# renjie-liang/HUAL

Hardware: AMD Instinct MI355X
Metric: train clips/sec (higher is better)
Workload: dtype f32 (fp16x3 / bf16x3 split-operand MFMA, fp32 accumulate); 1 GPU; Charades-STA SeqPAN train step (fwd+bwd+clip+AdamWD, dropout 0.2), batch 64/GPU, T=128, vdim=1024, L=20, C=8, dim=128, 8 heads, 2 attention layers, random init; ONE batch resident in HBM, batch assembly (hual_assemble_batch) outside the timed region; global_batch=64, T=128, vdim=1024, L=20, parallelism=dp1, launch=hipGraph, video_dtype=f32

## Files before the change

### hual_amd/csrc/embed.h

```cpp
#pragma once
#include "common.h"
#include "embed_args.h"
#include "gemm.h"

namespace hual {

struct EmbedLayout { int CP; size_t cemb, ball, yall, dxall, dfall, total; };
EmbedLayout embed_layout(int nrows, int C, int char_dim);
int embed_cpad(int char_dim);
int embed_gather_tasks(const EmbedArgs& a, int nrows);
int launch_embed_fwd(const EmbedArgs& a, int nrows, const DropCfg& drop, hipStream_t s);
void embed_dw_job(const EmbedArgs& a, int nrows, DwJob* dwjob);
int launch_embed_bwd(const EmbedArgs& a, const EmbedGrads& g, int nrows, const DropCfg& drop, hipStream_t s, DwJob* dwjob, bool finish = true);
int embed_finish_blocks(const EmbedArgs& a, int nrows);
int embed_finish_lds(const EmbedArgs& a);
int launch_embed_unpack(const EmbedArgs& a, const EmbedGrads& g, hipStream_t s);
int embed_unpack_tasks(const EmbedArgs& a);
int embed_unpack_cpad(const EmbedArgs& a);

}
```

### hual_amd/csrc/embed.hip

```cpp
#include "embed.h"
#include "mproj.h"
#include "philox.h"
#include "prof.h"

using namespace hual;

#include "embed_gather.h"

namespace hual {
static inline int cpad(int char_dim) { return (char_dim + 15) / 16 * 16; }
EmbedLayout embed_layout(int nrows, int C, int char_dim) {
  EmbedLayout l;
  const int CP = cpad(char_dim);
  const size_t M = (size_t)nrows * C;
  l.CP = CP;
  size_t off = 0;
  l.cemb = off; off += (M + 4) * CP;
  l.ball = off; off += NALL;
  l.yall = off; off += M * NALL;
  l.dxall = off; off += M * 4 * CP;
  l.dfall = off; off += (size_t)4 * CP * NALL + NALL;
  l.total = off;
  return l;
}
}

__global__ __launch_bounds__(256) void char_pool_kernel(EmbedArgs a, int nrows) {
  const int gid = blockIdx.x * 256 + threadIdx.x;
  if (gid >= nrows * NCH) return;
  const int row = gid / NCH, ch = gid - row * NCH;
  int k, chk;
  chan_to_kernel(ch, k, chk);
  const float* y = a.yall + (size_t)row * a.C * NALL + ch;
  float best = 0.f;
  int arg = -1;
  for (int p = 0; p + k <= a.C; ++p) {
    const float v = y[(size_t)p * NALL];
    if (v > best) { best = v; arg = p; }
  }
  a.cat[(size_t)row * a.ldcat + a.word_dim + ch] = best;
  a.char_arg[(size_t)row * NCH + ch] = arg;
}

__global__ __launch_bounds__(256) void char_pool_bwd_kernel(EmbedArgs a, EmbedGrads gr, DropCfg drop, int nrows, int CP,
                                                            int ntask_pool) {
  const int gid = blockIdx.x * 256 + threadIdx.x;
  const int C = a.C, wd = a.word_dim;
  if (gid < ntask_pool) {
    const int row = gid / NALL, col = gid - row * NALL;
    int arg = -1;
    float g = 0.f;
    if (col < NCH) {
      arg = a.char_arg[(size_t)row * NCH + col];
      if (arg >= 0) g = gr.dcat[(size_t)row * gr.lddcat + wd + col];
    }
    float* y = a.yall + (size_t)row * C * NALL + col;
    for (int p = 0; p < C; ++p) y[(size_t)p * NALL] = p == arg ? g : 0.f;
    return;
  }
  int x = gid - ntask_pool;
  const int ngw = wd >> 2;
  if (x < nrows * ngw) {
    const int row = x / ngw, c4 = x - row * ngw;
    const int wid = a.word_ids[row];
    float* dst = nullptr;
    if (wid == 1) dst = gr.dunk;
    else if (wid >= 2 && wid - 2 < gr.dword_rows) dst = gr.dword_table + (size_t)(wid - 2) * wd;
    if (dst) {
      float4 g = ld4(gr.dcat + (size_t)row * gr.lddcat + 4 * c4);
      if (drop.enabled) g = apply_drop4(drop, HUAL_SITE_WORD, (uint32_t)row, (uint32_t)c4, g);
      atomicAdd(dst + 4 * c4, g.x); atomicAdd(dst + 4 * c4 + 1, g.y);
      atomicAdd(dst + 4 * c4 + 2, g.z); atomicAdd(dst + 4 * c4 + 3, g.w);
    }
    return;
  }
  x -= nrows * ngw;
  if (x < 4 * CP * NALL + NALL) a.dfall[x] = 0.f;
}

__global__ __launch_bounds__(256) void embed_finish_kernel(EmbedArgs a, EmbedGrads gr, DropCfg drop, int nrows, int CP) {
  extern __shared__ float dT[];
  embed_finish_block(a, gr, drop, nrows, CP, blockIdx.x, dT);
}

__global__ __launch_bounds__(256) void embed_unpack_kernel(EmbedArgs a, EmbedGrads gr, int CP) {
  embed_unpack_task(a, gr, CP, blockIdx.x * 256 + threadIdx.x);
}

namespace hual {

static int check_args(const EmbedArgs& a) {
  HUAL_REQUIRE(a.C >= 4, "char_ids need at least 4 chars per word (conv width 4, VALID) - modules.py:33");
  HUAL_REQUIRE((a.word_dim % 4) == 0 && a.char_dim >= 1, "embed: word_dim must be a multiple of 4");
  HUAL_REQUIRE(a.cemb && a.wall_img && a.ball && a.yall && a.dxall && a.dfall, "embed: null scratch");
  return 0;
}

int embed_cpad(int char_dim) { return cpad(char_dim); }
int embed_gather_tasks(const EmbedArgs& a, int nrows) {
  const int CP = cpad(a.char_dim);
  return nrows * (a.word_dim / 4 + a.C * (CP / 4)) + 4 * CP + NALL;
}

int launch_embed_fwd(const EmbedArgs& a, int nrows, const DropCfg& drop, hipStream_t s) {
  int rc = check_args(a);
  if (rc) return rc;
  const int CP = cpad(a.char_dim);
  MProjArgs g{};
  g.R = nrows * a.C; g.MT = mproj_rows(g.R); g.nsteps = 1;
  MProjStep& st = g.s[0];
  st.A = a.cemb; st.lda = CP; st.rep = cdiv(4 * CP, 128); st.ktot = 4 * CP; st.kw = 4 * CP < 128 ? 4 * CP : 128; st.wimg = a.wall_img; st.wrows = 4 * CP;
  st.first = 1; st.last = 1; st.drop_site = -1; st.add_div = 1;
  st.bias = a.ball; st.out = a.yall; st.ldo = NALL; st.ncol = NALL;
  const int C = a.C;
  const int mtp = (g.MT + C - 1) / C * C;
  if ((C & (C - 1)) == 0 && C <= 16 && mtp <= 64) {
    g.MT = mtp;
    st.out = nullptr;
    g.pool_cat = a.cat; g.pool_ldcat = a.ldcat; g.pool_col0 = a.word_dim; g.pool_arg = a.char_arg; g.pool_C = C;
    return launch_mproj(&g, 1, drop, s);
  }
  rc = launch_mproj(&g, 1, drop, s);
  if (rc) return rc;
  HUAL_LAUNCH(0.0, 0.0, char_pool_kernel, dim3(cdiv(nrows * NCH, 256)), dim3(256), 0, s, a, nrows);
  HUAL_CHECK_HIP(hipGetLastError());
  return 0;
}

int embed_finish_blocks(const EmbedArgs& a, int nrows) { return cdiv(nrows * a.C, EF_ROWS); }
int embed_finish_lds(const EmbedArgs& a) { return (a.num_chars - 1) * a.char_dim * (int)sizeof(float); }
int launch_embed_bwd(const EmbedArgs& a, const EmbedGrads& g, int nrows, const DropCfg& drop, hipStream_t s, DwJob* dwjob, bool finish) {
  int rc = check_args(a);
  if (rc) return rc;
  HUAL_REQUIRE(dwjob != nullptr, "embed_bwd: null weight-gradient job");
  const int cd = a.char_dim, CP = cpad(cd), M = nrows * a.C;
  const int ntask_pool = nrows * NALL;
  const int ntail = nrows * (a.word_dim / 4) + 4 * CP * NALL + NALL;
  HUAL_LAUNCH(0.0, 0.0, char_pool_bwd_kernel, dim3(cdiv(ntask_pool + ntail, 256)), dim3(256), 0, s, a, g, drop, nrows, CP,
              ntask_pool);
  HUAL_CHECK_HIP(hipGetLastError());
  embed_dw_job(a, nrows, dwjob);
  HUAL_REQUIRE(a.wall_img_t != nullptr && cdiv(4 * CP, 128) <= MP_MAX, "embed_bwd: image of the transposed filter bank");
  MProjArgs j{};
  j.R = M; j.MT = mproj_rows(M); j.nsteps = cdiv(4 * CP, 128);
  for (int p = 0; p < j.nsteps; ++p) {
    MProjStep& st = j.s[p];
    st.A = a.yall; st.lda = NALL; st.kw = NALL; st.reuse = p > 0 ? 1 : 0; st.rep = 1;
    st.wimg = reinterpret_cast<const float*>(reinterpret_cast<const char*>(a.wall_img_t) + (size_t)p * HUAL_PACK_BLOCK_BYTES); st.wrows = NALL;
    st.first = 1; st.last = 1; st.drop_site = -1; st.add_div = 1;
    st.out = a.dxall + (size_t)p * 128; st.ldo = 4 * CP; st.ncol = 4 * CP - 128 * p < 128 ? 4 * CP - 128 * p : 128;
  }
  rc = launch_mproj(&j, 1, drop, s);
  if (rc) return rc;
  const size_t lds = (size_t)(a.num_chars - 1) * cd * sizeof(float);
  HUAL_REQUIRE(lds <= 64 * 1024, "embed_bwd: char table too large for the LDS accumulator");
  if (!finish) return 0;
  HUAL_LAUNCH(0.0, 0.0, embed_finish_kernel, dim3(cdiv(M, EF_ROWS)), dim3(256), lds, s, a, g, drop, nrows, CP);
  HUAL_CHECK_HIP(hipGetLastError());
  return 0;
}

void embed_dw_job(const EmbedArgs& a, int nrows, DwJob* dwjob) {
  const int CP = cpad(a.char_dim);
  dw_job_init(*dwjob);
  dwjob->npieces = 1;
  dwjob->A[0] = a.cemb; dwjob->lda[0] = CP; dwjob->kw[0] = 4 * CP; dwjob->dW[0] = a.dfall; dwjob->ldw = NALL;
  dwjob->dY = a.yall; dwjob->ldy = NALL; dwjob->M = nrows * a.C; dwjob->N = NALL;
  dwjob->db = a.dfall + (size_t)4 * CP * NALL;
}

int embed_unpack_tasks(const EmbedArgs& a) { return a.char_dim * 300 + NCH; }
int embed_unpack_cpad(const EmbedArgs& a) { return cpad(a.char_dim); }
int launch_embed_unpack(const EmbedArgs& a, const EmbedGrads& g, hipStream_t s) {
  const int cd = a.char_dim;
  const int n = cd * 300 + NCH;
  HUAL_LAUNCH(0.0, 0.0, embed_unpack_kernel, dim3(cdiv(n, 256)), dim3(256), 0, s, a, g, cpad(cd));
  HUAL_CHECK_HIP(hipGetLastError());
  return 0;
}

}
```

### hual_amd/csrc/embed_args.h

```cpp
#pragma once
#include "common.h"

namespace hual {

struct EmbedArgs {
  const int32_t* word_ids;
  const int32_t* char_ids;
  const float* word_table;
  const float* unk;
  const float* char_table;
  const float* filt[4];
  const float* fbias[4];
  float* cat; int ldcat;
  int32_t* char_arg;
  int word_dim, char_dim, C, num_chars;
  float* cemb; float* ball; float* yall; float* dxall; float* dfall;
  const float* wall_img; const float* wall_img_t;
};
struct EmbedGrads {
  const float* dcat; int lddcat;
  float* dunk; float* dchar_table; float* dfilt[4]; float* dfbias[4];
  float* dword_table; int dword_rows;
};

}
```

### hual_amd/csrc/prof.cpp

```cpp
#include <stdlib.h>
#include "prof.h"
#include <map>
#include <string>
#include <vector>
#include <string.h>
#include "../../include/hual_seqpan.h"

namespace hual {

namespace {
struct Rec { std::string name; hipEvent_t a, b; double flops, bytes; };
struct Agg { std::string name; int64_t launches = 0; double usec = 0.0, flops = 0.0, bytes = 0.0; };
struct State {
  bool on = false;
  std::vector<Rec> recs;
  std::vector<Agg> aggs;
};
thread_local State g_prof;

std::string clean(const char* s) {
  std::string n(s);
  while (!n.empty() && (n.front() == '(' || n.front() == ' ')) n.erase(n.begin());
  while (!n.empty() && (n.back() == ')' || n.back() == ' ')) n.pop_back();
  return n;
}
}

bool prof_on() { return g_prof.on; }
bool lds_poison_on() {
  static const bool on = getenv("HUAL_DEBUG_LDS_POISON") != nullptr && atoi(getenv("HUAL_DEBUG_LDS_POISON")) != 0;
  return on;
}

void prof_events(const char* name, double flops, double bytes, hipEvent_t* start, hipEvent_t* stop) {
  *start = *stop = nullptr;
  hipEvent_t a, b;
  if (hipEventCreate(&a) != hipSuccess) return;
  if (hipEventCreate(&b) != hipSuccess) { hipEventDestroy(a); return; }
  g_prof.recs.push_back(Rec{clean(name), a, b, flops, bytes});
  *start = a;
  *stop = b;
}

}

extern "C" {

int hual_prof_begin(void) {
  hual::g_prof.on = true;
  hual::g_prof.recs.clear();
  hual::g_prof.aggs.clear();
  return 0;
}

int hual_prof_end(void) {
  using namespace hual;
  g_prof.on = false;
  std::map<std::string, size_t> idx;
  g_prof.aggs.clear();
  for (auto& r : g_prof.recs) {
    hipEventSynchronize(r.b);
    float ms = 0.f;
    const bool ok = hipEventElapsedTime(&ms, r.a, r.b) == hipSuccess;
    auto it = idx.find(r.name);
    if (it == idx.end()) {
      it = idx.emplace(r.name, g_prof.aggs.size()).first;
      g_prof.aggs.push_back(Agg{r.name});
    }
    Agg& a = g_prof.aggs[it->second];
    if (ok) { a.launches += 1; a.usec += (double)ms * 1e3; a.flops += r.flops; a.bytes += r.bytes; }
    hipEventDestroy(r.a);
    hipEventDestroy(r.b);
  }
  g_prof.recs.clear();
  return (int)g_prof.aggs.size();
}

int hual_prof_get(int i, char* name, int name_cap, int64_t* launches, double* usec, double* flops, double* bytes) {
  using namespace hual;
  if (i < 0 || i >= (int)g_prof.aggs.size() || !name || name_cap < 1) return HUAL_ERR_INVALID;
  const Agg& a = g_prof.aggs[i];
  strncpy(name, a.name.c_str(), (size_t)name_cap - 1);
  name[name_cap - 1] = 0;
  if (launches) *launches = a.launches;
  if (usec) *usec = a.usec;
  if (flops) *flops = a.flops;
  if (bytes) *bytes = a.bytes;
  return 0;
}

int hual_prof_kernel_pipe(const char* kernel, int* pipe, int* passes) {
  if (!kernel || !pipe || !passes) return HUAL_ERR_INVALID;
  struct Row { const char* prefix; int pipe, passes; };
  static const Row rows[] = {
      {"conv_block_", HUAL_PIPE_MATRIX16, 3}, {"ln_proj", HUAL_PIPE_MATRIX16, 3}, {"da_post", HUAL_PIPE_MATRIX16, 3},
      {"da_mid_bwd", HUAL_PIPE_MATRIX16, 3},  {"ln2_mid_bwd", HUAL_PIPE_MATRIX16, 3}, {"mproj_", HUAL_PIPE_MATRIX16, 3},
      {"feature_", HUAL_PIPE_MATRIX16, 3},    {"dw_f16_", HUAL_PIPE_MATRIX16, 3},
      {"attn_", HUAL_PIPE_MATRIX16, 3},      {"cq_fwd_staged", HUAL_PIPE_MATRIX16, 3}, {"cq_bwd_staged", HUAL_PIPE_MATRIX16, 3},
      {"cq_fwd_wide", HUAL_PIPE_MATRIX16, 3}, {"cq_bwd_wide", HUAL_PIPE_MATRIX16, 3},
      {"cq_", HUAL_PIPE_MATRIX32, 1},
  };
  for (const Row& r : rows)
    if (strncmp(kernel, r.prefix, strlen(r.prefix)) == 0) { *pipe = r.pipe; *passes = r.passes; return 0; }
  *pipe = HUAL_PIPE_NONE; *passes = 0;
  return 0;
}

}
```

### hual_amd/csrc/seqpan.hip

```cpp
#include "attn.h"
#include "prof.h"
#include "cq.h"
#include "convblock.h"
#include "dablock.h"
#include "embed.h"
#include "gemm.h"
#include "heads.h"
#include "mproj.h"
#include "optim.h"
#include "params.h"
#include "rowops.h"
#include <stdlib.h>
#include <string.h>
#include <algorithm>
#include <unordered_map>
#include <vector>

namespace hual {
const char* last_error_cstr();
}
using namespace hual;

namespace {

// ... 377 lines not shown
  AlignPool& ap = f.align;
  ap.F2 = cqf; ap.F1 = cqf; ap.inner = (lab && !c.dry) ? lab->inner_labels : nullptr;
  ap.tpre = r("align.tpre", B, D); ap.vpre = r("align.vpre", B, D);
  ap.that = r("align.tv", B, 2 * D); ap.vhat = ap.that + D; ap.ld = 2 * D;
  f.fuse = r.actv("fuse"); f.outputs = r.actv("outputs");
  f.probs = r("match.probs", c.rs.Nv, 4); f.match_part = r("match.part", (size_t)match_fwd_blocks(c.rs.Nv), 2);
  f.d_that = r("d.align.that", B, D); f.d_vhat = r("d.align.vhat", B, D);
  f.align_scratch = r("align.scratch", (size_t)2 * B, B); f.align_rows = r("align.rowloss", B, 1);
  return f;
}
MatchArgs match_args(const Ctx& c, const CoreBufs& k, const FuseBufs& f, const hual_labels* lab, const hual_run_opts* opt) {
  MatchArgs ma{};
  ma.fuse = f.fuse; ma.Wm = c.p(c.pm.match.k); ma.bm = c.p(c.pm.match.b); ma.E = c.p(c.pm.label_emb);
  ma.labels = (lab && !c.dry) ? lab->match_labels : nullptr;
  ma.outputs = f.outputs; ma.loss_acc = k.loss_acc;
  if (!c.cfg->no_gumbel) { ma.rng = opt->rng_state; ma.inv_tau = 1.0f / c.cfg->tau; }
  return ma;
}

struct FeBufs {
  float *x0, *a, *mean, *rstd, *qkv; uint8_t* kb4;
  CbBufs cb;
  float* att; AttnJob job; float *res, *l2, *mean2, *rstd2, *out; uint8_t *kb6, *kb7, *kb8;
};
FeBufs fe_bufs(const Res& r, int ps) {
  const Ctx& c = r.c;
  const int D = HUAL_D, Nv = c.rs.Nv;
  const std::string t = "fe" + std::to_string(ps);
  FeBufs b{};
  b.x0 = r.actv(t + ".x0"); b.a = r.actv(t + ".a");
  b.mean = r(t + ".ln1.mean", Nv, 1); b.rstd = r(t + ".ln1.rstd", Nv, 1);
  b.qkv = r(t + ".qkv", Nv, 3 * D); b.kb4 = r.bits(t + ".kb4", Nv);
  b.cb = cb_bufs(r, t, b.x0, Nv);
  b.att = r.actv(t + ".att");
  AttnJob& a = b.job;
  attn_job_init(a);
  a.Q = b.qkv; a.ldq = 3 * D; a.K = b.qkv + D; a.V = b.qkv + 2 * D; a.ldkv = 3 * D; a.O = b.att; a.ldo = D;
  a.B = c.B; a.Tq = c.T; a.Tk = c.T; a.qrow0 = 0; a.krow0 = 0; a.qmask = c.rs.rowmask; a.kmask = c.rs.rowmask;
  a.drop_site = HUAL_SITE_FE + 16 * ps + 5;
  set_dmask(r, a, t + ".dm");
  b.res = r.actv(t + ".res"); b.l2 = r.actv(t + ".l2");
  b.mean2 = r(t + ".ln2.mean", Nv, 1); b.rstd2 = r(t + ".ln2.rstd", Nv, 1);
  b.out = r.actv(t + ".out");
  b.kb6 = r.bits(t + ".kb6", Nv); b.kb7 = r.bits(t + ".kb7", Nv); b.kb8 = r.bits(t + ".kb8", Nv);
  return b;
}

struct HeadBufs { float *fn[2], *mean, *rstd, *h[2], *d_logit[2], *dz[2], *part[2], *loc_part; };
HeadBufs head_bufs(const Res& r) {
  const Ctx& c = r.c;
  const int D = HUAL_D, Nv = c.rs.Nv, B = c.B;
  HeadBufs b{};
  b.fn[0] = r.actv("head.sfn"); b.fn[1] = r.actv("head.efn");
  b.mean = r("head.mean", (size_t)2 * Nv, 1); b.rstd = r("head.rstd", (size_t)2 * Nv, 1);
  b.h[0] = r.actv("head.hs"); b.h[1] = r.actv("head.he");
  b.d_logit[0] = r("d.s_logit", B, c.T); b.d_logit[1] = r("d.e_logit", B, c.T);
  b.dz[0] = r.actv("d.head.zs"); b.dz[1] = r.actv("d.head.ze");
  b.part[0] = r("head.part.s", (size_t)B * 2, D); b.part[1] = r("head.part.e", (size_t)B * 2, D);
  b.loc_part = r("loc.part", B, 1);
  return b;
}

void fill_da_ln_proj(Ctx& c, LnProjArgs& lp, int li) {
  const int D = HUAL_D;
  const DualAttnP& d = c.pm.da[li];
  const DaLnBufs n = da_ln_bufs(Res{c, true}, li);
  lp = LnProjArgs{};
  lp.g1 = c.p(d.ln1.g); lp.b1 = c.p(d.ln1.b); lp.y1 = n.ln1; lp.drop_site1 = -1; lp.pre_site = -1;
  lp.g2 = c.p(d.lnt.g); lp.b2 = c.p(d.lnt.b); lp.y2 = n.lnt; lp.mean = n.mean; lp.rstd = n.rstd;
  lp.nproj = 5; lp.R = c.rs.R; lp.Nv = c.rs.Nv; lp.MT = ln_proj_rows(c.rs.R, c.rs.Nv); lp.drop_row0 = 0;
  const DenseP* pr[5] = {&d.query, &d.f_key, &d.f_value, &d.t_key, &d.t_value};
  float* outs[5] = {n.qkv, n.qkv + D, n.qkv + 2 * D, n.ktvt, n.ktvt + D};
  for (int k = 0; k < 5; ++k) {
    lp.wimg[k] = c.timg(pr[k]->k); lp.bias[k] = c.p(pr[k]->b); lp.out[k] = outs[k]; lp.ldo[k] = k < 3 ? 3 * D : 2 * D; lp.src[k] = k < 3 ? 0 : 1;
    lp.out_site[k] = -1;
  }
}

bool cb_no_tail() {
  static const bool no_tail = getenv("HUAL_CB_NO_TAIL") != nullptr && atoi(getenv("HUAL_CB_NO_TAIL")) != 0;
  return no_tail;
}

float* conv_block_fwd(Ctx& c, const CbBufs& b, const ConvBlockP& cp, const RowSpace& rs, int site0,
                      const float* pos_src = nullptr, const float* pos = nullptr, LnProjArgs* tail = nullptr, bool* tail_done = nullptr) {
  CbFwdArgs a{};
  a.x0 = pos_src ? pos_src : b.x[0]; a.pos = pos; a.x0_out = pos_src ? b.x[0] : nullptr;
  a.MT = conv_block_fused_rows(rs.R, rs.Nq > 0 ? rs.Nv : 0); a.drop_row0 = 0;
  for (int i = 0; i < 4; ++i) {
    CbLayerFwd& L = a.l[i];
    L.c = b.c[i];
    L.y = c.debug_taps ? b.y[i] : nullptr;
    L.relu_bits = b.rb[i]; L.keep_bits = b.kb[i]; L.xout = b.x[i + 1]; L.mean = b.mean[i]; L.rstd = b.rstd[i];
    L.ln_g = c.p(cp.ln[i].g); L.ln_b = c.p(cp.ln[i].b); L.dw = c.p(cp.dw[i]);
    L.wimg = c.timg(cp.pw[i]); L.bias = c.p(cp.b[i]);
    L.drop_site = site0 + i;
  }
  const bool fuse = tail && c.sel_stage < 0 && !cb_no_tail();
  if (tail) tail->x = b.x[4];
  if (tail_done) *tail_done = fuse;
  if (c.live()) c.chk(launch_conv_block_fwd(a, rs, c.drop, c.stream, fuse ? tail : nullptr));
  return b.x[4];
}

float* conv_block_bwd(Ctx& c, const CbBufs& b, float* dx, const ConvBlockP& cp, const RowSpace& rs) {
  const int R = rs.R;
  const std::string dt = "d." + b.tag;
  CbBwdArgs a{};
  a.dx_in = dx; a.relu_bits3 = b.rb[3]; a.keep_bits3 = b.kb[3];
  a.dx_out = c.buf(dt + ".x0", R, HUAL_D);
  a.MT = conv_block_fused_rows_bwd(R, rs.Nq > 0 ? rs.Nv : 0); a.drop_row0 = 0;
  const int nblk = conv_block_bwd_blocks(R, rs.Nq > 0 ? rs.Nv : 0);
  for (int i = 3; i >= 0; --i) {
    CbLayerBwd& L = a.l[i];
    L.ln_g = c.p(cp.ln[i].g); L.ln_b = c.p(cp.ln[i].b); L.dw = c.p(cp.dw[i]);
    L.wimg_t = c.nimg(cp.pw[i]);
    L.x = b.x[i]; L.mean = b.mean[i]; L.rstd = b.rstd[i];
    L.relu_prev = i > 0 ? b.rb[i - 1] : nullptr; L.keep_prev = i > 0 ? b.kb[i - 1] : nullptr;
    L.dz = c.buf(dt + ".z" + std::to_string(i), R, HUAL_D);
    L.dz_prev = i > 0 ? c.buf(dt + ".z" + std::to_string(i - 1), R, HUAL_D) : nullptr;
    L.part = c.buf("part." + std::to_string(c.part_seq++), (size_t)nblk * 9, HUAL_D);
    ColsumJob cj{};
    cj.src = L.part; cj.nblk = nblk; cj.nvec = 9;
    for (int k = 0; k < 7; ++k) cj.dst[k] = c.g(cp.dw[i]) + k * HUAL_D;
    cj.dst[7] = c.g(cp.ln[i].g); cj.dst[8] = c.g(cp.ln[i].b);
    if (c.active) c.colsum.push_back(cj);
    c.push_dw(mkdw(b.c[i], HUAL_D, HUAL_D, L.dz, HUAL_D, R, c.g(cp.pw[i]), c.g(cp.b[i])));
  }
  if (c.live()) c.chk(launch_conv_block_bwd(a, rs, c.drop, c.stream));
  return a.dx_out;
}


void fwd_prologue(Ctx& c, const CoreBufs& k, const InputBufs& in, EmbedArgs& ea, const hual_batch* bt, const hual_labels* lab,
                  const hual_run_opts* opt) {
  if (c.dry || !c.ok()) return;
  const ParamMap& pm = c.pm;
  std::vector<uint32_t> offs, boffs; std::vector<int> Ks; std::vector<uint8_t> needs;
  for (const auto& d : c.dense) { offs.push_back((uint32_t)d.off); Ks.push_back(d.K); boffs.push_back((uint32_t)d.boff); needs.push_back(d.need); }
  offs.push_back(c.wall_off); Ks.push_back(c.wall_K); boffs.push_back(c.wall_boff);
  needs.push_back(HUAL_PACK_T | HUAL_PACK_N);
  fill_embed_args(c, ea, bt, in.cat, c.catw(), in.char_arg, in.embed_scratch);
  PackExtra ex{};
  ex.lens = bt->video_seq_len; ex.word_ids = bt->word_ids; ex.rowmask = k.rowmask; ex.loss_acc = k.loss_acc; ex.B = c.B; ex.T = c.T; ex.L = c.L;
  ex.zero_ptr = (lab && opt->grads_prezero && opt->prezero_token) ? opt->grads_prezero : nullptr;
  ex.zero_n = (size_t)((pm.total + 3) & ~(size_t)3);
  ex.E = lab ? c.p(pm.label_emb) : nullptr; ex.lambda = c.cfg->match_lambda; ex.dE_ortho = k.ortho_dE;
  ex.gather_tasks = (c.stage_on(ST_INPUT) && c.word_table) ? embed_gather_tasks(ea, c.rs.Nq) : 0;
  ex.gather_rows = c.rs.Nq; ex.emb = ea; ex.drop = c.drop;
  ex.wall_K = c.wall_K; ex.wall_off = c.wall_off; ex.wall_boff = c.wall_boff;
  if (c.novf) { ex.ovf = k.ovf; ex.novf = c.novf; }
  c.chk(launch_pack_weights(offs.data(), Ks.data(), boffs.data(), (int)offs.size(), c.P, c.PKF, c.stream, &ex,
                            c.PKT, c.want_bwd ? c.PKN : nullptr, needs.data()));
  if (opt->prezero_token) *opt->prezero_token = (ex.zero_ptr && c.ok()) ? (uint64_t)(uintptr_t)ex.zero_ptr : 0;
}

void fwd_input(Ctx& c, const InputBufs& in, const EmbedArgs& ea, const hual_batch* bt) {
  const ParamMap& pm = c.pm;
  const int Nv = c.rs.Nv, Nq = c.rs.Nq, R = c.rs.R, D = HUAL_D, catw = c.catw();
  c.stage(ST_INPUT);
  if (!c.live()) return;
  c.chk(launch_embed_fwd(ea, Nq, c.drop, c.stream));
  if (!c.ok()) return;
  float* x = in.x0;
  if (c.ksplit) {
    const int qks = ((catw + 3) / 4 + 63) & ~63;
// ... 408 lines not shown
  float* dz2 = c.act(dt + ".z2");
  c.push_dw(mkdw(b.l2, D, D, dz2, D, R, c.g(d.dense2.k), c.g(d.dense2.b)));
  float *d_res = c.act(dt + ".res"), *dz1 = c.act(dt + ".z1"), *d_sc = c.act(dt + ".sc"), *d_val = c.act(dt + ".val");
  float *d_ln1a = c.act(dt + ".ln1a"), *d_g = c.act(dt + ".g"), *dz_sg = c.act(dt + ".zsg"), *dz_xg = c.act(dt + ".zxg");
  float *d_sv = c.act(dt + ".s"), *d_xv = c.act(dt + ".x"), *d_satt = c.act(dt + ".s_att"), *d_xatt = c.act(dt + ".x_att");
  const bool dz2_ready = li < c.cfg->attn_layer - 1 && c.sel_stage < 0;
  c.push_dw(mkdw(b.mha, D, D, dz1, D, R, c.g(d.dense1.k), c.g(d.dense1.b)));
  for (int k = 0; k < 2; ++k) {
    DwJob j = mkdw(b.n.ln1, D, D, k == 0 ? d_sc : d_val, D, R, c.g(k == 0 ? d.bl1_d1 : d.bl2_d1), c.g(k == 0 ? d.bl1_b : d.bl2_b));
    j.npieces = 2; j.A[1] = b.gd; j.lda[1] = D; j.kw[1] = D; j.dW[1] = c.g(k == 0 ? d.bl1_d2 : d.bl2_d2);
    c.push_dw(j);
  }
  c.push_dw(mkdw(b.o, D, D, d_g, D, R, c.g(d.guided.k), c.g(d.guided.b)));
  c.push_dw(mkdw(b.sv, D, D, dz_sg, D, R, c.g(d.s_gate.k), c.g(d.s_gate.b)));
  c.push_dw(mkdw(b.xv, D, D, dz_xg, D, R, c.g(d.x_gate.k), c.g(d.x_gate.b)));
  c.push_dw(mkdw(b.s_att, D, D, d_sv, D, R, c.g(d.s_dense.k), c.g(d.s_dense.b)));
  c.push_dw(mkdw(b.x_att, D, D, d_xv, D, R, c.g(d.x_dense.k), c.g(d.x_dense.b)));
  {
    LnProjBwdArgs lb{};
    lb.nsteps = 1; lb.lda[0] = D; lb.wimg_t[0] = c.nimg(d.dense2.k); lb.dst[0] = 0;
    if (dz2_ready) { lb.A[0] = dz2; }
    else { lb.A[0] = dx; lb.a_bits[0] = b.kb4; lb.a_save[0] = dz2; }
    lb.dy1_bits = b.kb3; lb.x = b.res; lb.mean = b.mean2; lb.rstd = b.rstd2; lb.g1 = c.p(d.ln2.g); lb.add1 = dx;
    lb.dx = d_res; lb.dz = dz1; lb.dz_bits = b.kb2; lb.R = R; lb.Nv = Nv; lb.drop_row0 = 0;
    DaMidBwdArgs mb{};
    mb.dz1 = dz1; mb.gate = b.gate; mb.val = b.val; mb.sg = b.sg; mb.xg = b.xg; mb.sv = b.sv; mb.xv = b.xv;
    const size_t wo[10] = {d.dense1.k, d.bl1_d1, d.bl2_d1, d.bl1_d2, d.bl2_d2, d.guided.k, d.s_gate.k, d.x_gate.k, d.s_dense.k, d.x_dense.k};
    for (int k = 0; k < 10; ++k) mb.w[k] = c.nimg(wo[k]);
    mb.d_sc = d_sc; mb.d_val = d_val; mb.d_ln1a = d_ln1a; mb.d_g = d_g; mb.dz_sg = dz_sg; mb.dz_xg = dz_xg; mb.d_sv = d_sv; mb.d_xv = d_xv;
    mb.d_satt = d_satt; mb.d_xatt = d_xatt; mb.R = R; mb.Nv = Nv;
    c.ln2_mid_bwd(lb, mb, c.g(d.ln2.g), c.g(d.ln2.b));
  }
  float *dq_self = c.act(dt + ".q_self"), *dq_cross = c.act(dt + ".q_cross");
  float *d_qkv = c.buf(dt + ".qkv", R, 3 * D), *d_ktvt = c.buf(dt + ".ktvt", R, 2 * D);
  AttnJob a[4];
  for (int k = 0; k < 4; ++k) {
    const bool cross = k & 1;
    a[k] = b.att[k];
    a[k].lddo = D; a[k].lddq = D; a[k].dO = cross ? d_xatt : d_satt; a[k].dQ = cross ? dq_cross : dq_self;
    a[k].dK = cross ? d_ktvt : d_qkv + D; a[k].dV = cross ? d_ktvt + D : d_qkv + 2 * D; a[k].lddkv = cross ? 2 * D : 3 * D;
  }
  c.attn_bwd(a, 4);
  const float* As[6] = {dq_self, dq_cross, d_qkv + D, d_qkv + 2 * D, d_ktvt, d_ktvt + D};
  const int lds_[6] = {D, D, 3 * D, 3 * D, 2 * D, 2 * D};
  const DenseP* pr[6] = {&d.query, &d.query, &d.f_key, &d.f_value, &d.t_key, &d.t_value};
  for (int k = 0; k < 6; ++k) c.push_dw(mkdw(k < 4 ? b.n.ln1 : b.n.lnt, D, D, As[k], lds_[k], R, c.g(pr[k]->k), c.g(pr[k]->b)));
  float* d_xin = c.act(dt + ".in");
  float* nz = nullptr; const uint8_t* nz_bits = nullptr;
  if (li > 0) { nz = c.act("d.da" + std::to_string(li - 1) + ".z2"); nz_bits = r.bits("da" + std::to_string(li - 1) + ".kb4", R); }
  {
    LnProjBwdArgs lb{};
    lb.nsteps = 6;
    for (int k = 0; k < 6; ++k) { lb.A[k] = As[k]; lb.lda[k] = lds_[k]; lb.wimg_t[k] = c.nimg(pr[k]->k); lb.dst[k] = k < 4 ? 0 : 1; }
    lb.add_dy1 = d_ln1a; lb.x = xin; lb.mean = b.n.mean; lb.rstd = b.n.rstd; lb.g1 = c.p(d.ln1.g); lb.g2 = c.p(d.lnt.g);
    lb.add1 = d_res; lb.dx = d_xin; lb.dz = nz; lb.dz_bits = nz_bits; lb.R = R; lb.Nv = Nv; lb.drop_row0 = 0;
    c.ln_proj_bwd(lb, c.g(d.ln1.g), c.g(d.ln1.b), c.g(d.lnt.g), c.g(d.lnt.b));
  }
  return d_xin;
}

bool bwd_input(Ctx& c, const InputBufs& in, float* d_x0, float* const fe_dx0[2], const hual_batch* bt, EmbedArgs& ea, EmbedGrads& eg) {
  const ParamMap& pm = c.pm;
  const int D = HUAL_D, Nv = c.rs.Nv, Nq = c.rs.Nq, catw = c.catw();
  c.stage(ST_ALWAYS);
  PosBwdJob pj[2];
  int npj = 0;
  if (!c.dry && c.stage_on(ST_INPUT)) pj[npj++] = PosBwdJob{{d_x0, nullptr}, c.g(pm.pos), 1, 1};
  if (!c.dry && c.stage_on(ST_PRED)) pj[npj++] = PosBwdJob{{fe_dx0[1], fe_dx0[0]}, c.g(pm.fe_pos), 1, 0};
  const bool pos_rides = c.sel_stage < 0;
  if (c.live() && npj && !pos_rides) c.chk(launch_pos_bwd(pj, npj, c.rs, c.stream));
  c.stage(ST_INPUT);
  float* d_lin = c.act("d.lin");
  LnBwd a{};
  a.x = in.lin; a.mean = in.lin_mean; a.rstd = in.lin_rstd; a.R = c.rs.R; a.dy1 = d_x0; a.g1 = c.p(pm.vln.g);
  a.dx = d_lin; a.split = Nv; a.g1_hi = c.p(pm.qln.g);
  c.ln_bwd_split(a, c.g(pm.vln.g), c.g(pm.vln.b), c.g(pm.qln.g), c.g(pm.qln.b), pj, pos_rides ? npj : 0);
  DwJob j = mkdw(c.dry ? nullptr : reinterpret_cast<const float*>(bt->video), c.cfg->vdim, c.cfg->vdim, d_lin, D, Nv, c.g(pm.vconv.k), c.g(pm.vconv.b));
  j.a_drop_site = HUAL_SITE_VIDEO; j.a_drop_row0 = 0;
  j.a_bf16 = (!c.dry && bt->video_dtype == HUAL_DTYPE_BF16) ? 1 : 0;
  j.a_keep = in.vkeep; j.ld_keep = (c.cfg->vdim + 7) / 8;
  c.push_dw(j);
  c.push_dw(mkdw(in.cat, catw, catw, d_lin + (size_t)Nv * D, D, Nq, c.g(pm.qconv.k), c.g(pm.qconv.b)));
  float* d_cat = c.buf("d.cat", Nq, catw);
  if (c.live()) {
    if (cdiv(catw, 128) > MP_MAX) { c.chk(fail(-1, "invalid argument: internal: query_conv1d image")); return c.active; }
    MProjArgs pr = margs(Nq);
    pr.nsteps = cdiv(catw, 128);
    for (int p = 0; p < pr.nsteps; ++p) {
      const float* img = c.nimg(pm.qconv.k, p);
      pr.s[p] = p == 0 ? mstep(d_lin + (size_t)Nv * D, D, D, img, D, true, true) : mstep_reuse(img, D, true, true);
      mstep_out(pr.s[p], d_cat + (size_t)p * D, catw, nullptr, std::min(D, catw - p * D));
    }
    c.chk(launch_mproj(&pr, 1, c.drop, c.stream));
  }
  set_embed_scratch(ea, in.embed_scratch, Nq, c.C, c.cfg->char_dim);
  ea.word_dim = c.cfg->word_dim; ea.char_dim = c.cfg->char_dim; ea.C = c.C; ea.num_chars = c.cfg->num_chars;
  DwJob embed_dw;
  embed_dw_job(ea, Nq, &embed_dw);
  if (c.live()) {
    fill_embed_args(c, ea, bt, in.cat, catw, in.char_arg, in.embed_scratch);
    eg.dcat = d_cat; eg.lddcat = catw; eg.dunk = c.g(pm.unk); eg.dchar_table = c.g(pm.char_table);
    if (pm.word_table != (size_t)-1) { eg.dword_table = c.g(pm.word_table); eg.dword_rows = c.cfg->num_words - 2; }
    for (int i = 0; i < 4; ++i) { eg.dfilt[i] = c.g(pm.filt[i]); eg.dfbias[i] = c.g(pm.fbias[i]); }
    c.chk(launch_embed_bwd(ea, eg, Nq, c.drop, c.stream, &embed_dw, false));
  }
  c.push_dw(embed_dw);
  return c.active;
}

void bwd_flush(Ctx& c, const EmbedArgs& ea, const EmbedGrads& eg, bool input_ran) {
  c.stage(ST_ALWAYS);
  flush_dw(c);
  EmbedUnpack eu{};
  const bool unpack = !c.dry && input_ran && c.active;
  if (unpack) {
    eu.a = ea; eu.g = eg; eu.CP = embed_unpack_cpad(ea); eu.ntasks = embed_unpack_tasks(ea);
    eu.finish_blocks = embed_finish_blocks(ea, c.rs.Nq); eu.finish_lds = embed_finish_lds(ea); eu.nrows = c.rs.Nq; eu.drop = c.drop;
  }
  c.flush_colsum(unpack ? &eu : nullptr);
}

int backward_graph(Ctx& c, const hual_batch* bt, const hual_labels* lab, const hual_run_opts* opt) {
  const Res r{c, false};
  c.dwjobs.clear(); c.colsum.clear(); c.part_seq = 0;
  c.stage(ST_ALWAYS);
  const CoreBufs core = core_bufs(r);
  const InputBufs in = input_bufs(r);
  const CqStage cq = cq_bufs(r, r.act("da" + std::to_string(c.cfg->attn_layer - 1) + ".out"));
  const FuseBufs fu = fuse_bufs(r, cq.feats, lab);
  const HeadBufs hd = head_bufs(r);
  {
    const bool prezeroed = !c.dry && opt->prezero_token && *opt->prezero_token == (uint64_t)(uintptr_t)c.G && c.sel_stage < 0;
    if (!c.dry && opt->prezero_token) *opt->prezero_token = 0;
    if (c.live() && !prezeroed) c.chk(launch_zero(c.G, c.pm.total, c.stream));
  }
  c.stage(ST_PRED);
  const HeadGrads hg = bwd_heads(c, hd, fu.outputs);
  float* fe_dx0[2] = {nullptr, nullptr};
  fe_dx0[1] = bwd_fe(c, 1, hd, hg.d_fn[1], nullptr);
  fe_dx0[0] = bwd_fe(c, 0, hd, hg.d_fn[0], fe_dx0[1]);
  float* d_cqf = bwd_fuse(c, core, fu, hd, cq.feats, fe_dx0[0], hg.d_out, lab, opt);
  float* dx = bwd_cq(c, cq, d_cqf);
  for (int li = c.cfg->attn_layer - 1; li >= 0; --li) dx = bwd_da(c, li, dx);
  c.stage(ST_CONV);
  float* d_x0 = conv_block_bwd(c, cb_bufs(r, "cb", in.x0, c.rs.R), dx, c.pm.cb, c.rs);
  EmbedArgs ea{}; EmbedGrads eg{};
  const bool input_ran = bwd_input(c, in, d_x0, fe_dx0, bt, ea, eg);
  bwd_flush(c, ea, eg, input_ran);
  return c.rc;
}

int plan(Ctx& c, const hual_cfg* cfg, int B, int T, int L, int C) {
  int rc = setup_ctx(c, cfg, B, T, L, C);
  if (rc) return rc;
  c.dry = true;
  c.base = nullptr;
  hual_run_opts o{};
  rc = forward_graph(c, nullptr, nullptr, nullptr, &o);
  if (rc) return rc;
  return backward_graph(c, nullptr, nullptr, &o);
}

}

extern "C" {

int hual_seqpan_validate(const hual_cfg* cfg) {
  HUAL_REQUIRE(cfg != nullptr, "null cfg");
  return validate_cfg(*cfg);
}

#define HUAL_DW_TABLE_JOBS 256
uint64_t hual_seqpan_dw_table_bytes(void) { return 4 * dw_table_words(HUAL_DW_TABLE_JOBS); }

int hual_seqpan_param_count(const hual_cfg* cfg, uint64_t* padded_floats, uint64_t* count) {
  HUAL_REQUIRE(cfg != nullptr, "null cfg");
  ParamMap pm;
  int rc = build_param_map(*cfg, pm);
  if (rc) return rc;
  if (padded_floats) *padded_floats = pm.total;
  if (count) *count = pm.count;
  return 0;
}

int hual_seqpan_param_table(const hual_cfg* cfg, hual_param_entry* out, int max_entries) {
  HUAL_REQUIRE(cfg != nullptr, "null cfg");
  ParamMap pm;
// ... 271 lines not shown
```

Measured before the change: 53840 clips/s.

## Fuse query-conv backward, char-pool backward and filter dX projection into one kernel

Adds a fused embed_chain_bwd kernel that computes d_cat from d_lin via the query_conv1d weight image, scatters word-embedding gradients, builds the max-pool backward rows and multiplies them by the transposed filter bank, all inside LDS per tile of words. It replaces three launches (the mproj for d_cat, char_pool_bwd and the mproj for dxall), removing their round-trips through global memory and the launch gaps. The cost is a larger LDS footprint and lower occupancy for this small stage, plus an env var to fall back to the old path.

```diff
diff --git a/hual_amd/csrc/embed.h b/hual_amd/csrc/embed.h
--- a/hual_amd/csrc/embed.h
+++ b/hual_amd/csrc/embed.h
@@ -11,7 +11,9 @@
 int embed_gather_tasks(const EmbedArgs& a, int nrows);
 int launch_embed_fwd(const EmbedArgs& a, int nrows, const DropCfg& drop, hipStream_t s);
 void embed_dw_job(const EmbedArgs& a, int nrows, DwJob* dwjob);
-int launch_embed_bwd(const EmbedArgs& a, const EmbedGrads& g, int nrows, const DropCfg& drop, hipStream_t s, DwJob* dwjob, bool finish = true);
+bool embed_chain_fits(const EmbedArgs& a, int catw);
+int launch_embed_bwd(const EmbedArgs& a, const EmbedGrads& g, int nrows, const DropCfg& drop, hipStream_t s, DwJob* dwjob, bool finish = true,
+                     const EmbedChain* chain = nullptr);
 int embed_finish_blocks(const EmbedArgs& a, int nrows);
 int embed_finish_lds(const EmbedArgs& a);
 int launch_embed_unpack(const EmbedArgs& a, const EmbedGrads& g, hipStream_t s);
diff --git a/hual_amd/csrc/embed.hip b/hual_amd/csrc/embed.hip
--- a/hual_amd/csrc/embed.hip
+++ b/hual_amd/csrc/embed.hip
@@ -2,6 +2,7 @@
 #include "mproj.h"
 #include "philox.h"
 #include "prof.h"
+#include "tilecore.h"
 
 using namespace hual;
 
@@ -76,6 +77,103 @@
   }
   x -= nrows * ngw;
   if (x < 4 * CP * NALL + NALL) a.dfall[x] = 0.f;
+}
+
+#define EC_ROWS 64
+#define EC_QB 4
+#define EC_WB 2
+#define EC_TS (EC_QB * 128)
+#define EC_LDS (2 * 16 * 256 + 2 * EC_ROWS * 256 + 16 * EC_TS * 4 + (16 + EC_ROWS + 16) * 4)
+__global__ __launch_bounds__(CB_THREADS) void embed_chain_bwd_kernel(EmbedArgs a, EmbedGrads gr, EmbedChain ch, DropCfg drop, int nrows, int CP) {
+  extern __shared__ __attribute__((aligned(16))) char ec_lds[];
+  char* SA = ec_lds;
+  char* SY = SA + 2 * 16 * 256;
+  float* dcat = reinterpret_cast<float*>(SY + 2 * EC_ROWS * 256);
+  float* ainvA = dcat + 16 * EC_TS;
+  float* ainvY = ainvA + 16;
+  int* wid = reinterpret_cast<int*>(ainvY + EC_ROWS);
+  const int lane = threadIdx.x & 63, wave = threadIdx.x >> 6;
+  const int l32 = threadIdx.x & 31, grp = threadIdx.x >> 5, col = 4 * l32;
+  const int j = lane & 15, g = lane >> 4, ecol = 16 * wave + 4 * g;
+  const int C = a.C, wd = a.word_dim, W = ch.W;
+  {
+    const int n = 4 * CP * NALL + NALL;
+    for (int i = blockIdx.x * CB_THREADS + threadIdx.x; i < n; i += gridDim.x * CB_THREADS) st1f_global(a.dfall + i, 0.f);
+  }
+  const int w0 = xcd_tile(blockIdx.x, gridDim.x) * W;
+  if (w0 >= nrows) return;
+  const int nw = min(W, nrows - w0), nr = nw * C;
+  const float4 nv = ld4_global(ch.dlin + (size_t)min(w0 + grp, nrows - 1) * HUAL_D + col);
+  TfW wq[EC_QB];
+#pragma unroll
+  for (int p = 0; p < EC_QB; ++p) tf_load_w_if(wq[p], ch.qimg[p], p < ch.nqb, wave, lane);
+  float4 ca[4];
+#pragma unroll
+  for (int u = 0; u < 4; ++u) {
+    const int word = min(w0 + (grp + 16 * u) / C, nrows - 1);
+    ca[u] = ld4_global(a.char_arg + (size_t)word * NCH + min(col, NCH - 4));
+  }
+  const int widv = a.word_ids[min(w0 + (int)(threadIdx.x & 15), nrows - 1)];
+  {
+    const float inv = cb_store_operand(SA, SA + 16 * 256, grp, l32, grp < nw ? nv : f4zero());
+    if (l32 == 0) ainvA[grp] = grp < nw ? inv : 0.f;
+    if (threadIdx.x < 16) wid[threadIdx.x] = widv;
+  }
+  lds_barrier();
+#pragma unroll
+  for (int p = 0; p < EC_QB; ++p) {
+    f32x4 accp[1];
+    tf_mma<1, 16 * 256>(SA, wq[p], lane, accp);
+    const float ir = ainvA[j];
+    *reinterpret_cast<float4*>(dcat + j * EC_TS + 128 * p + ecol) =
+        make_float4(fmaf(accp[0][0], ir, 0.f), fmaf(accp[0][1], ir, 0.f), fmaf(accp[0][2], ir, 0.f), fmaf(accp[0][3], ir, 0.f));
+  }
+  TfW ww[EC_WB];
+#pragma unroll
+  for (int p = 0; p < EC_WB; ++p)
+    tf_load_w_if(ww[p], reinterpret_cast<const char*>(a.wall_img_t) + (size_t)min(p, ch.nwb - 1) * HUAL_PACK_BLOCK_BYTES, p < ch.nwb, wave, lane);
+  lds_barrier();
+  const int ngw = wd >> 2;
+  for (int x = threadIdx.x; x < nw * ngw; x += CB_THREADS) {
+    const int row = x / ngw, c4 = x - row * ngw;
+    const int id = wid[row];
+    float* dst = nullptr;
+    if (id == 1) dst = gr.dunk;
+    else if (id >= 2 && id - 2 < gr.dword_rows) dst = gr.dword_table + (size_t)(id - 2) * wd;
+    if (dst) {
+      float4 v = *reinterpret_cast<const float4*>(dcat + row * EC_TS + 4 * c4);
+      if (drop.enabled) v = apply_drop4(drop, HUAL_SITE_WORD, (uint32_t)(w0 + row), (uint32_t)c4, v);
+      atomic_add_global(dst + 4 * c4, v.x); atomic_add_global(dst + 4 * c4 + 1, v.y);
+      atomic_add_global(dst + 4 * c4 + 2, v.z); atomic_add_global(dst + 4 * c4 + 3, v.w);
+    }
+  }
+#pragma unroll
+  for (int u = 0; u < 4; ++u) {
+    const int lr = grp + 16 * u, word = lr / C, p = lr - word * C;
+    const bool valid = lr < nr;
+    float4 v = f4zero();
+    if (valid && col < NCH) {
+      const float4 gv = *reinterpret_cast<const float4*>(dcat + word * EC_TS + wd + col);
+      v = make_float4(__float_as_int(ca[u].x) == p ? gv.x : 0.f, __float_as_int(ca[u].y) == p ? gv.y : 0.f,
+                      __float_as_int(ca[u].z) == p ? gv.z : 0.f, __float_as_int(ca[u].w) == p ? gv.w : 0.f);
+    }
+    if (valid) st4_global(a.yall + ((size_t)w0 * C + lr) * NALL + col, v);
+    const float inv = cb_store_operand(SY, SY + EC_ROWS * 256, lr, l32, v);
+    if (l32 == 0) ainvY[lr] = valid ? inv : 0.f;
+  }
+  lds_barrier();
+#pragma unroll
+  for (int p = 0; p < EC_WB; ++p) {
+    f32x4 accp[4];
+    tf_mma<4, EC_ROWS * 256>(SY, ww[p], lane, accp);
+#pragma unroll
+    for (int rt = 0; rt < 4; ++rt) {
+      const int lr = 16 * rt + j;
+      const float ir = ainvY[lr];
+      const float4 v = make_float4(fmaf(accp[rt][0], ir, 0.f), fmaf(accp[rt][1], ir, 0.f), fmaf(accp[rt][2], ir, 0.f), fmaf(accp[rt][3], ir, 0.f));
+      if (lr < nr && 128 * p + ecol < 4 * CP) st4_global(a.dxall + ((size_t)w0 * C + lr) * 4 * CP + 128 * p + ecol, v);
+    }
+  }
 }
 
 __global__ __launch_bounds__(256) void embed_finish_kernel(EmbedArgs a, EmbedGrads gr, DropCfg drop, int nrows, int CP) {
@@ -129,11 +227,35 @@
 
 int embed_finish_blocks(const EmbedArgs& a, int nrows) { return cdiv(nrows * a.C, EF_ROWS); }
 int embed_finish_lds(const EmbedArgs& a) { return (a.num_chars - 1) * a.char_dim * (int)sizeof(float); }
-int launch_embed_bwd(const EmbedArgs& a, const EmbedGrads& g, int nrows, const DropCfg& drop, hipStream_t s, DwJob* dwjob, bool finish) {
+bool embed_chain_fits(const EmbedArgs& a, int catw) {
+  return a.C <= EC_ROWS && cdiv(catw, 128) <= EC_QB && cdiv(4 * cpad(a.char_dim), 128) <= EC_WB && a.wall_img_t != nullptr;
+}
+int launch_embed_bwd(const EmbedArgs& a, const EmbedGrads& g, int nrows, const DropCfg& drop, hipStream_t s, DwJob* dwjob, bool finish,
+                     const EmbedChain* chain) {
   int rc = check_args(a);
   if (rc) return rc;
   HUAL_REQUIRE(dwjob != nullptr, "embed_bwd: null weight-gradient job");
   const int cd = a.char_dim, CP = cpad(cd), M = nrows * a.C;
+  if (chain) {
+    const int catw = a.word_dim + NCH;
+    HUAL_REQUIRE(embed_chain_fits(a, catw) && chain->dlin && chain->nqb == cdiv(catw, 128), "embed_bwd: shape outside the fused chain");
+    for (int p = 0; p < chain->nqb; ++p) HUAL_REQUIRE(chain->qimg[p] != nullptr, "embed_bwd: image of query_conv1d");
+    EmbedChain ch = *chain;
+    ch.W = EC_ROWS / a.C < 16 ? EC_ROWS / a.C : 16;
+    ch.nwb = cdiv(4 * CP, 128);
+    const double flops = 2.0 * nrows * 128.0 * catw + 2.0 * M * 128.0 * 4.0 * CP;
+    const double bytes = 4.0 * (nrows * (128.0 + NCH + 1.0) + M * (128.0 + 4.0 * CP) + 128.0 * (catw + 4.0 * CP) + 4.0 * CP * NALL + NALL);
+    HUAL_DYN_LDS(embed_chain_bwd_kernel, EC_LDS);
+    HUAL_LAUNCH(flops, bytes, embed_chain_bwd_kernel, dim3(xcd_round8(cdiv(nrows, ch.W))), dim3(CB_THREADS), EC_LDS, s, a, g, ch, drop, nrows, CP);
+    HUAL_CHECK_HIP(hipGetLastError());
+    embed_dw_job(a, nrows, dwjob);
+    const size_t lds = (size_t)(a.num_chars - 1) * cd * sizeof(float);
+    HUAL_REQUIRE(lds <= 64 * 1024, "embed_bwd: char table too large for the LDS accumulator");
+    if (!finish) return 0;
+    HUAL_LAUNCH(0.0, 0.0, embed_finish_kernel, dim3(cdiv(M, EF_ROWS)), dim3(256), lds, s, a, g, drop, nrows, CP);
+    HUAL_CHECK_HIP(hipGetLastError());
+    return 0;
+  }
   const int ntask_pool = nrows * NALL;
   const int ntail = nrows * (a.word_dim / 4) + 4 * CP * NALL + NALL;
   HUAL_LAUNCH(0.0, 0.0, char_pool_bwd_kernel, dim3(cdiv(ntask_pool + ntail, 256)), dim3(256), 0, s, a, g, drop, nrows, CP,
diff --git a/hual_amd/csrc/embed_args.h b/hual_amd/csrc/embed_args.h
--- a/hual_amd/csrc/embed_args.h
+++ b/hual_amd/csrc/embed_args.h
@@ -22,5 +22,10 @@
   float* dunk; float* dchar_table; float* dfilt[4]; float* dfbias[4];
   float* dword_table; int dword_rows;
 };
+struct EmbedChain {
+  const float* dlin;
+  const float* qimg[4]; int nqb;
+  int W, nwb;
+};
 
 }
diff --git a/hual_amd/csrc/prof.cpp b/hual_amd/csrc/prof.cpp
--- a/hual_amd/csrc/prof.cpp
+++ b/hual_amd/csrc/prof.cpp
@@ -95,6 +95,7 @@
   static const Row rows[] = {
       {"conv_block_", HUAL_PIPE_MATRIX16, 3}, {"ln_proj", HUAL_PIPE_MATRIX16, 3}, {"da_post", HUAL_PIPE_MATRIX16, 3},
       {"da_mid_bwd", HUAL_PIPE_MATRIX16, 3},  {"ln2_mid_bwd", HUAL_PIPE_MATRIX16, 3}, {"mproj_", HUAL_PIPE_MATRIX16, 3},
+      {"embed_chain_bwd", HUAL_PIPE_MATRIX16, 3},
       {"feature_", HUAL_PIPE_MATRIX16, 3},    {"dw_f16_", HUAL_PIPE_MATRIX16, 3},
       {"attn_", HUAL_PIPE_MATRIX16, 3},      {"cq_fwd_staged", HUAL_PIPE_MATRIX16, 3}, {"cq_bwd_staged", HUAL_PIPE_MATRIX16, 3},
       {"cq_fwd_wide", HUAL_PIPE_MATRIX16, 3}, {"cq_bwd_wide", HUAL_PIPE_MATRIX16, 3},
diff --git a/hual_amd/csrc/seqpan.hip b/hual_amd/csrc/seqpan.hip
--- a/hual_amd/csrc/seqpan.hip
+++ b/hual_amd/csrc/seqpan.hip
@@ -483,6 +483,11 @@
   return no_tail;
 }
 
+bool embed_no_chain() {
+  static const bool no_chain = getenv("HUAL_EMBED_NO_CHAIN") != nullptr && atoi(getenv("HUAL_EMBED_NO_CHAIN")) != 0;
+  return no_chain;
+}
+
 float* conv_block_fwd(Ctx& c, const CbBufs& b, const ConvBlockP& cp, const RowSpace& rs, int site0,
                       const float* pos_src = nullptr, const float* pos = nullptr, LnProjArgs* tail = nullptr, bool* tail_done = nullptr) {
   CbFwdArgs a{};
@@ -1057,7 +1062,11 @@
   c.push_dw(j);
   c.push_dw(mkdw(in.cat, catw, catw, d_lin + (size_t)Nv * D, D, Nq, c.g(pm.qconv.k), c.g(pm.qconv.b)));
   float* d_cat = c.buf("d.cat", Nq, catw);
-  if (c.live()) {
+  set_embed_scratch(ea, in.embed_scratch, Nq, c.C, c.cfg->char_dim);
+  ea.word_dim = c.cfg->word_dim; ea.char_dim = c.cfg->char_dim; ea.C = c.C; ea.num_chars = c.cfg->num_chars;
+  if (c.live()) fill_embed_args(c, ea, bt, in.cat, catw, in.char_arg, in.embed_scratch);
+  const bool chain = c.live() && c.sel_stage < 0 && !embed_no_chain() && embed_chain_fits(ea, catw);
+  if (c.live() && !chain) {
     if (cdiv(catw, 128) > MP_MAX) { c.chk(fail(-1, "invalid argument: internal: query_conv1d image")); return c.active; }
     MProjArgs pr = margs(Nq);
     pr.nsteps = cdiv(catw, 128);
@@ -1068,16 +1077,18 @@
     }
     c.chk(launch_mproj(&pr, 1, c.drop, c.stream));
   }
-  set_embed_scratch(ea, in.embed_scratch, Nq, c.C, c.cfg->char_dim);
-  ea.word_dim = c.cfg->word_dim; ea.char_dim = c.cfg->char_dim; ea.C = c.C; ea.num_chars = c.cfg->num_chars;
   DwJob embed_dw;
   embed_dw_job(ea, Nq, &embed_dw);
   if (c.live()) {
-    fill_embed_args(c, ea, bt, in.cat, catw, in.char_arg, in.embed_scratch);
     eg.dcat = d_cat; eg.lddcat = catw; eg.dunk = c.g(pm.unk); eg.dchar_table = c.g(pm.char_table);
     if (pm.word_table != (size_t)-1) { eg.dword_table = c.g(pm.word_table); eg.dword_rows = c.cfg->num_words - 2; }
     for (int i = 0; i < 4; ++i) { eg.dfilt[i] = c.g(pm.filt[i]); eg.dfbias[i] = c.g(pm.fbias[i]); }
-    c.chk(launch_embed_bwd(ea, eg, Nq, c.drop, c.stream, &embed_dw, false));
+    EmbedChain ch{};
+    if (chain) {
+      ch.dlin = d_lin + (size_t)Nv * D; ch.nqb = cdiv(catw, 128);
+      for (int p = 0; p < ch.nqb; ++p) ch.qimg[p] = c.nimg(pm.qconv.k, p);
+    }
+    c.chk(launch_embed_bwd(ea, eg, Nq, c.drop, c.stream, &embed_dw, false, chain ? &ch : nullptr));
   }
   c.push_dw(embed_dw);
   return c.active;
```

After: 54320 clips/s (median of 6 runs). About the same (+0.9%).
